# arnaucube/fhe-study

Measured on AMD Instinct MI355X. Metric: NTT/s (N=2^16, 64-bit q) per node; achieved HBM GB/s vs roofline, higher is better.
Workload: dtype u64

## Files before the change

### fhe-study_amd/csrc/bfv32.hip

```cpp
#include "bfv32.hpp"
#include "ntt32_big.hpp"

#include <type_traits>

namespace fhe {

__device__ __forceinline__ u32 mont32(u32 x, u32 y, u32 p, u32 pinv_neg) {
    const u64 t = (u64)x * y;
    const u32 m = (u32)t * pinv_neg;
    return (u32)((t + (u64)m * p) >> 32);
}
__device__ __forceinline__ u64 crt2(u32 rA, u32 rB, u32 pA, u32 pB, Tw32 crt) {
    const u32 rAb = csub_u32(rA, pB);
    const u32 diff = rB - rAb + pB;
    const u32 h = csub_u32(mul_shoup32(diff, crt, pB), pB);
    return (u64)rA + (u64)pA * h;
}

#ifndef FHE_B32_INV_T
#define FHE_B32_INV_T 2
#endif
#ifndef FHE_B32_INV_R
#define FHE_B32_INV_R 1
#endif
#ifndef FHE_B32_FWD_PRELOAD
#define FHE_B32_FWD_PRELOAD 1
#endif
#ifndef FHE_B32_FWD_WAVES
#define FHE_B32_FWD_WAVES 4
#endif
#ifndef FHE_B32_RELIN_WAVES
#define FHE_B32_RELIN_WAVES 4
#endif
#ifndef FHE_B32_FWD2_WAVES
#define FHE_B32_FWD2_WAVES 6
#endif
#ifndef FHE_B32_FWD2_PRELOAD
#define FHE_B32_FWD2_PRELOAD 0
#endif
#ifndef FHE_B32_FWD3_WAVES
#define FHE_B32_FWD3_WAVES 4
#endif
#ifndef FHE_B32_FWD3_RELOAD
#define FHE_B32_FWD3_RELOAD 0
#endif
constexpr int fwd_waves(int npr) { return npr == 2 ? FHE_B32_FWD2_WAVES : npr == 3 ? FHE_B32_FWD3_WAVES : FHE_B32_FWD_WAVES; }
constexpr bool fwd_reload(int npr) { return npr == 3 && FHE_B32_FWD3_RELOAD != 0; }
constexpr bool fwd_preload(int npr) { return npr == 2 ? FHE_B32_FWD2_PRELOAD != 0 : FHE_B32_FWD_PRELOAD != 0; }
#ifndef FHE_B32_PARK_LDS
#define FHE_B32_PARK_LDS 1
#endif
constexpr int kRelinWps = 4;
#ifndef FHE_B32_INV_LOOSE
#define FHE_B32_INV_LOOSE 1
#endif
template <int MODE> constexpr int last_in_of() { return (FHE_B32_INV_LOOSE && MODE != 0) ? 8 : 2; }
template <int MODE, int LB>
__device__ __forceinline__ void inv_block(u32 (&v)[1][16], u32 *lds, const Tw32 *ltw, const Tw32 *gtw, u32 tf, u32 p, u32 p2, u32 bq, u32 blk) {
    if constexpr (FHE_B32_INV_LOOSE && MODE != 0) inv_big_loose<LB, MODE == 2, last_in_of<MODE>()>(v, lds, ltw, gtw, tf, p, bq, 1u, blk);
    else if constexpr (MODE == 0) inv_big<LB>(v, lds, ltw, gtw, tf, p, p2, 1u, blk);
    else if constexpr (MODE == 1) inv_big_direct<LB, false>(v, lds, ltw, gtw, tf, p, p2, 1u, blk);
    else inv_big_direct<LB, true>(v, lds, ltw, gtw, tf, p, p2, 1u, blk);
}
template <int LB>
struct Blk {
    using C = Big32<LB>;
    static constexpr u32 M = C::M, TH = C::TH;
    static constexpr size_t LDS(int tables) { return C::TILE_BYTES + (size_t)tables * C::TW_BYTES; }
    static constexpr int park_lds(int tables, int words, int wps) {
        const long wgs = (4L * wps * 64) / (long)TH;
        const long budget = 160L * 1024 / (wgs < 1 ? 1 : wgs) - 1024;
        const long k = (budget - (long)LDS(tables)) / (8L * (long)TH);
        return k < 0 ? 0 : (k > words ? words : (int)k);
    }
    static constexpr size_t LDS_PARKED(int tables, int words, int wps) { return LDS(tables) + (size_t)park_lds(tables, words, wps) * 8 * TH; }
    static __device__ __forceinline__ Tw32 *table(unsigned char *smem, int i) { return reinterpret_cast<Tw32 *>(smem + C::TILE_BYTES + i * C::TW_BYTES); }
};

template <int LB, int NPR, bool WORD32, bool BELOWP = false>
__global__ __launch_bounds__((Big32<LB>::TH), fwd_waves(NPR)) void bfv32_forward_kernel(Bfv32Args a) {
    static_assert(!BELOWP || WORD32, "words below a 27-bit prime are below 2^32");
    using C = Big32<LB>;
    using K = Blk<LB>;
    extern __shared__ __attribute__((aligned(16))) unsigned char smem_raw[];
    u32 *lds = reinterpret_cast<u32 *>(smem_raw);
    const u32 tf = threadIdx.x;
    const u64 g8 = blockIdx.x / 16;
    const u32 r16 = blockIdx.x % 16;
    const u64 row = g8 * 8 + (r16 & 7u);
    const u32 blk = r16 >> 3;
    if (row >= a.rows) return;
#pragma unroll
    for (int i = 0; i < NPR; i++) stage_tw32_block<C::TH>(K::table(smem_raw, i), a.t.tw_fwd[NPR == 1 ? blockIdx.y : i], C::LTW_N, tf, 1u, blk);
    const u64 *__restrict__ src = a.src + row * K::M;
    typename std::conditional<WORD32, u32, u64>::type x[16];
#pragma unroll
    for (int k = 0; k < 16; k++) x[k] = (typename std::conditional<WORD32, u32, u64>::type)src[(u32)k * C::TH + tf];
    __syncthreads();
#pragma unroll
    for (int i = 0; i < NPR; i++) {
        const u32 pr = NPR == 1 ? blockIdx.y : (u32)i;
        const u32 p = a.t.p[pr], p2 = 2u * p;
        if constexpr (fwd_reload(NPR)) {
            if (i > 0) {
                u64 sa = reinterpret_cast<u64>(src);
// ... 28 lines not shown
    }
}
template <int KIN>
__device__ __forceinline__ void last_stage(u32 &lo, u32 &hi, Tw32 ni, Tw32 w1ni, u32 p) {
    static_assert(2 * KIN <= 16, "the sum of two values below KIN p stays in a word (p < 2^32 / 25)");
    const u32 s = lo + hi, d = lo - hi + (u32)KIN * p;
    lo = csub_u32(mul_shoup32(s, ni, p), p);
    hi = csub_u32(mul_shoup32(d, w1ni, p), p);
}

__device__ __forceinline__ u64 zq_scale_round_int(u64 N, u64 q, u64 mu) {
    u64 a = __umul64hi(N, mu);
    u64 f = N - a * q;
    if (f >= q) { f -= q; a += 1; }
    if (f >= q) { f -= q; a += 1; }
    a += (2 * f >= q);
    u64 r = a - __umul64hi(a, mu) * q;
    r = r >= q ? r - q : r;
    return r >= q ? r - q : r;
}

#ifndef FHE_B32_INT_TAIL
#define FHE_B32_INT_TAIL 1
#endif
__device__ __forceinline__ u64 zq_from_f64_small(double ef, double qf, double qinv, u32 q) {
    const double e = round(ef);
#if FHE_B32_INT_TAIL
    const double k = floor(e * qinv);
    int r = (int)fma(-k, qf, e);
    r += (r >> 31) & (int)q;
    return (u64)min((u32)r, (u32)r - q);
#else
    const double k = rint(e * qinv);
    double r = fma(-k, qf, e);
    r = r < 0.0 ? r + qf : r;
    r = r < 0.0 ? r + qf : r;
    r = r >= qf ? r - qf : r;
    return (u64)(u32)r;
#endif
}
__device__ __forceinline__ double exact_quotient(double N, double den, double rden) {
    const double q0 = N * rden;
    const double r = fma(-q0, den, N);
    return fma(r, rden, q0);
}
template <bool SMALL>
__device__ __forceinline__ u64 scale_round(const Bfv32Args &a, long long v) {
    const double N = a.numf * (double)v;
    const double x = a.rdenf != 0.0 ? exact_quotient(N, a.denf, a.rdenf) : N / a.denf;
    if constexpr (SMALL) return zq_from_f64_small(x, (double)a.q, a.qinvf, (u32)a.q);
    else return zq_from_f64_mu(a.q, a.qmu, round(x));
}

template <int LB, bool INT, bool SMALL>
__global__ __launch_bounds__((Big32<LB>::TH), 4) void bfv32_tensor_inverse_kernel(Bfv32Args a) {
    using C = Big32<LB>;
    using K = Blk<LB>;
    extern __shared__ __attribute__((aligned(16))) unsigned char smem_raw[];
    u32 *lds = reinterpret_cast<u32 *>(smem_raw);
    const u32 tf = threadIdx.x;
    const u64 g8 = blockIdx.x / 24;
    const u32 r24 = blockIdx.x % 24;
    const u64 b = g8 * 8 + (r24 & 7u);
    const u32 which = r24 >> 3;
    if (b >= a.batch) return;
#pragma unroll
    for (int i = 0; i < 4; i++) stage_tw32_block<C::TH>(K::table(smem_raw, i), a.t.tw_inv[i >> 1], C::LTW_N, tf, 1u, (u32)(i & 1));
    __syncthreads();
    auto prime = [&](auto prc) __attribute__((always_inline)) {
        constexpr int pr = decltype(prc)::value;
        const u32 p = a.t.p[pr], p2 = 2u * p, pn = a.pinv_neg[pr];
        const u32 *__restrict__ fw = a.fw + (((u64)pr * a.rows) << (LB + 1));
        auto block = [&](u32 blk, u32 (&v)[1][16]) __attribute__((always_inline)) {
            const u32 off = blk * K::M + tf * 4u;
            auto rowp = [&](u32 w) { return fw + (((u64)w * a.batch + b) << (LB + 1)) + off; };
            const u32 *__restrict__ ra = rowp(which == 2 ? 1 : 0), *__restrict__ rb = rowp(which == 0 ? 2 : 3);
            const u32 *__restrict__ rc = rowp(1), *__restrict__ rd = rowp(2);
#pragma unroll
            for (int j = 0; j < 4; j++) {
                const uint4 xa = *reinterpret_cast<const uint4 *>(ra + j * (K::M / 4)), xb = *reinterpret_cast<const uint4 *>(rb + j * (K::M / 4));
                u32 t[4] = {mont32(xa.x, xb.x, p, pn), mont32(xa.y, xb.y, p, pn), mont32(xa.z, xb.z, p, pn), mont32(xa.w, xb.w, p, pn)};
                if (which == 1) {
                    const uint4 xc = *reinterpret_cast<const uint4 *>(rc + j * (K::M / 4)), xd = *reinterpret_cast<const uint4 *>(rd + j * (K::M / 4));
                    t[0] = csub_u32(t[0] + mont32(xc.x, xd.x, p, pn), p2); t[1] = csub_u32(t[1] + mont32(xc.y, xd.y, p, pn), p2);
                    t[2] = csub_u32(t[2] + mont32(xc.z, xd.z, p, pn), p2); t[3] = csub_u32(t[3] + mont32(xc.w, xd.w, p, pn), p2);
                }
                v[0][4 * j] = t[0]; v[0][4 * j + 1] = t[1]; v[0][4 * j + 2] = t[2]; v[0][4 * j + 3] = t[3];
            }
#ifndef FHE_B32_ABLATE_INV
            inv_block<FHE_B32_INV_T, LB>(v, lds, K::table(smem_raw, 2 * pr + (int)blk), a.t.tw_inv[pr], tf, p, p2, a.t.bq[pr], blk);
#endif
        };
        u32 v0[1][16], v1[1][16];
        block(0u, v0);
        block(1u, v1);
        const Tw32 ni = a.ninv_mont[pr], w1ni = a.w1ninv_mont[pr];
        u64 parked = 0;
        u32 tfe = tf;
        asm volatile("" : "+v"(tfe));
        u64 *po = a.out + ((u64)which * a.batch + b) * K::M + tfe;
        u64 psa = reinterpret_cast<u64>(po);
        asm volatile("" : "+v"(psa));
        const gu64 *ps = reinterpret_cast<const gu64 *>(psa);
        if constexpr (pr == 1) parked = ps[0];
#pragma unroll
        for (int k = 0; k < 16; k++) {
            u32 rl = v0[0][k], rh = v1[0][k];
            last_stage<last_in_of<FHE_B32_INV_T>()>(rl, rh, ni, w1ni, p);
            if constexpr (pr == 0) {
                po[(u32)k * C::TH] = ((u64)rh << 32) | rl;
            } else {
                const u32 loA = (u32)parked, hiA = (u32)(parked >> 32);
                if (k + 1 < 16) parked = ps[(u32)(k + 1) * C::TH];
                const long long lo = (long long)crt2(loA, rl, a.t.p[0], a.t.p[1], a.t.crt);
                const long long hi = (long long)crt2(hiA, rh, a.t.p[0], a.t.p[1], a.t.crt);
#ifndef FHE_B32_ABLATE_EPI
                u64 zl, zh;
                if constexpr (INT) {
                    zl = zq_scale_round_int(a.int_num * (u64)lo, a.q, a.qmu);
                    zh = zq_scale_round_int(a.int_num * (u64)hi, a.q, a.qmu);
                } else {
                    zl = scale_round<SMALL>(a, lo);
                    zh = scale_round<SMALL>(a, hi);
                }
#else
                const u64 zl = (u64)lo, zh = (u64)hi;
#endif
                po[(u32)k * C::TH] = zl >= zh ? zl - zh : (a.q + zl) - zh;
                __builtin_amdgcn_sched_barrier(0);
            }
        }
    };
    prime(std::integral_constant<int, 0>{});
    prime(std::integral_constant<int, 1>{});
}

template <int LB, bool SMALL>
__global__ __launch_bounds__((Big32<LB>::TH), FHE_B32_RELIN_WAVES) void bfv32_relin_inverse_kernel(Bfv32Args a) {
    using C = Big32<LB>;
    using K = Blk<LB>;
    extern __shared__ __attribute__((aligned(16))) unsigned char smem_raw[];
    u32 *lds = reinterpret_cast<u32 *>(smem_raw);
    const u32 tf = threadIdx.x;
    const u64 g8 = blockIdx.x / 16;
    const u32 r16 = blockIdx.x % 16;
    const u64 b = g8 * 8 + (r16 & 7u);
    const u32 o = r16 >> 3;
    if (b >= a.batch) return;
#pragma unroll
    for (int i = 0; i < 6; i++) stage_tw32_block<C::TH>(K::table(smem_raw, i), a.t.tw_inv[i >> 1], C::LTW_N, tf, 1u, (u32)(i & 1));
    __syncthreads();
    const u64 off = ((u64)o * a.batch + b) * K::M + tf;
    u64 *park0 = a.park + off, *park1 = park0 + 2 * a.batch * K::M;
    auto prime = [&](auto prc) __attribute__((always_inline)) {
        constexpr int pr = decltype(prc)::value;
        const u32 p = a.t.p[pr], p2 = 2u * p, pn = a.pinv_neg[pr];
        auto block = [&](u32 blk, u32 (&v)[1][16]) __attribute__((always_inline)) {
            const u32 bo = blk * K::M + tf * 4u;
            const u32 *__restrict__ rx = a.x + (((u64)pr * a.batch + b) << (LB + 1)) + bo;
            const u32 *__restrict__ rk = a.key + (((u64)pr * 2 + o) << (LB + 1)) + bo;
#pragma unroll
            for (int j = 0; j < 4; j++) {
                const uint4 xa = *reinterpret_cast<const uint4 *>(rx + j * (K::M / 4)), xb = *reinterpret_cast<const uint4 *>(rk + j * (K::M / 4));
                v[0][4 * j] = mont32(xa.x, xb.x, p, pn); v[0][4 * j + 1] = mont32(xa.y, xb.y, p, pn);
                v[0][4 * j + 2] = mont32(xa.z, xb.z, p, pn); v[0][4 * j + 3] = mont32(xa.w, xb.w, p, pn);
            }
#ifndef FHE_B32_ABLATE_INV
            inv_block<FHE_B32_INV_R, LB>(v, lds, K::table(smem_raw, 2 * pr + (int)blk), a.t.tw_inv[pr], tf, p, p2, a.t.bq[pr], blk);
#endif
        };
        u32 v0[1][16], v1[1][16];
        block(0u, v0);
        block(1u, v1);
        const Tw32 ni = a.ninv_mont[pr], w1ni = a.w1ninv_mont[pr];
        u64 pk0 = 0, pk1 = 0;
        u64 psa0 = reinterpret_cast<u64>(park0), psa1 = reinterpret_cast<u64>(park1);
        asm volatile("" : "+v"(psa0), "+v"(psa1));
        const gu64 *ps0 = reinterpret_cast<const gu64 *>(psa0), *ps1 = reinterpret_cast<const gu64 *>(psa1);
        constexpr int KL = FHE_B32_PARK_LDS ? K::park_lds(6, 16, kRelinWps) : 0;
        u64 *lpark = reinterpret_cast<u64 *>(smem_raw + K::LDS(6)) + tf;
        auto park0_load = [&](int k) __attribute__((always_inline)) { return k < KL ? lpark[(u32)k * C::TH] : ps0[(u32)k * C::TH]; };
        if constexpr (pr >= 1) pk0 = park0_load(0);
        if constexpr (pr == 2) pk1 = ps1[0];
#pragma unroll
        for (int k = 0; k < 16; k++) {
            u32 r2[2] = {v0[0][k], v1[0][k]};
            last_stage<last_in_of<FHE_B32_INV_R>()>(r2[0], r2[1], ni, w1ni, p);
            if constexpr (pr == 0) {
                if (k < KL) lpark[(u32)k * C::TH] = ((u64)r2[1] << 32) | r2[0];
                else park0[(u32)k * C::TH] = ((u64)r2[1] << 32) | r2[0];
            } else if constexpr (pr == 1) {
                const u32 g0[2] = {(u32)pk0, (u32)(pk0 >> 32)};
                if (k + 1 < 16) pk0 = park0_load(k + 1);
                u32 g1[2];
#pragma unroll
                for (int h = 0; h < 2; h++) {
                    const u32 d = r2[h] - csub_u32(g0[h], p) + p;
                    g1[h] = csub_u32(mul_shoup32(d, a.t.crt, p), p);
                }
                park1[(u32)k * C::TH] = ((u64)g1[1] << 32) | g1[0];
            } else {
                const u32 g0[2] = {(u32)pk0, (u32)(pk0 >> 32)}, g1[2] = {(u32)pk1, (u32)(pk1 >> 32)};
                if (k + 1 < 16) { pk0 = park0_load(k + 1); pk1 = ps1[(u32)(k + 1) * C::TH]; }
                long long R2[2];
#pragma unroll
                for (int h = 0; h < 2; h++) {
                    const u32 a0 = csub_u32(csub_u32(g0[h], p), p);
                    const u32 d = r2[h] - a0 + p;
                    const u32 e = csub_u32(mul_shoup32(d, a.t.crt_ac, p), p);
                    const u32 b1 = csub_u32(g1[h], p);
                    const u32 v2 = csub_u32(mul_shoup32(e - b1 + p, a.t.crt_bc, p), p);
                    R2[h] = (long long)((u64)g0[h] + (u64)a.t.p[0] * g1[h] + a.t.P * v2);
                }
                const long long lo = R2[0], hi = R2[1];
#ifndef FHE_B32_ABLATE_EPI
                const u64 zl = scale_round<SMALL>(a, lo);
                const u64 zh = scale_round<SMALL>(a, hi);
#else
                const u64 zl = (u64)lo, zh = (u64)hi;
#endif
                u64 v = zl >= zh ? zl - zh : (a.q + zl) - zh;
                const u64 at = off + (u32)k * C::TH;
                v += a.addend[at];
                if (v >= a.q) v -= a.q;
                a.out[at] = v;
                __builtin_amdgcn_sched_barrier(0);
            }
        }
    };
    prime(std::integral_constant<int, 0>{});
    prime(std::integral_constant<int, 1>{});
    prime(std::integral_constant<int, 2>{});
}

static unsigned bits_of64(uint64_t x) { unsigned b = 0; while (x) { b++; x >>= 1; } return b; }

bool bfv32_shape_supported(uint64_t q, uint64_t n, uint64_t pq) {
    if (n < 1024 || n > 8192 || (n & (n - 1)) || q < 2) return false;
    const unsigned ln = bits_of64(n - 1), bq = bits_of64(q - 1);
    if (2 * bq + ln + 1 > 54) return false;
    if (pq && (pq < q || bq + bits_of64(pq - 1) + ln > 82)) return false;
    return true;
}

template <typename K>
static hipError_t launch_big(K kernel, const char *name, int lp, size_t lds, unsigned th, u64 grid, const Bfv32Args &a, hipStream_t st,
                             unsigned gridy = 1) {
    if (grid == 0) return hipSuccess;
    if (grid > 0x7fffffffull) return hipErrorInvalidValue;
    if (hipError_t e = allow_big_lds((const void *)kernel, lds)) return e;
    KernelTimer kt(name, lp, st);
    hipLaunchKernelGGL(kernel, dim3((unsigned)grid, gridy), dim3(th), lds, st, a);
    return hipGetLastError();
}
#define FHE_BIG_SWITCH(KERNEL, NAME, GRID, GRIDY, TABLES, PARKW, WPS)                                                               \
    switch (a.log_n2) {                                                                                                      \
        case 11: return launch_big(KERNEL<10>, NAME, 11, Blk<10>::LDS_PARKED(TABLES, PARKW, WPS), Big32<10>::TH, GRID, a, st, GRIDY); \
        case 12: return launch_big(KERNEL<11>, NAME, 12, Blk<11>::LDS_PARKED(TABLES, PARKW, WPS), Big32<11>::TH, GRID, a, st, GRIDY); \
        case 13: return launch_big(KERNEL<12>, NAME, 13, Blk<12>::LDS_PARKED(TABLES, PARKW, WPS), Big32<12>::TH, GRID, a, st, GRIDY); \
        case 14: return launch_big(KERNEL<13>, NAME, 14, Blk<13>::LDS_PARKED(TABLES, PARKW, WPS), Big32<13>::TH, GRID, a, st, GRIDY); \
    }                                                                                                                        \
    return hipErrorNotSupported;

template <int LB> static constexpr auto bfv32_forward2 = bfv32_forward_kernel<LB, 2, true>;
template <int LB> static constexpr auto bfv32_forward3 = bfv32_forward_kernel<LB, 3, true>;
template <int LB> static constexpr auto bfv32_forward2b = bfv32_forward_kernel<LB, 2, true, true>;
template <int LB> static constexpr auto bfv32_forward3b = bfv32_forward_kernel<LB, 3, true, true>;
template <int LB> static constexpr auto bfv32_forward1w = bfv32_forward_kernel<LB, 1, false>;
hipError_t launch_bfv32_forward(const Bfv32Args &a, hipStream_t st) {
    const u64 grid = 16 * ((a.rows + 7) / 8);
    if (a.primes == 2 && a.word32 && a.below_p) { FHE_BIG_SWITCH(bfv32_forward2b, "bfv32_forward", grid, 1, 2, 0, 4) }
    if (a.primes == 3 && a.word32 && a.below_p) { FHE_BIG_SWITCH(bfv32_forward3b, "bfv32_forward3", grid, 1, 3, 0, 4) }
    if (a.primes == 2 && a.word32) { FHE_BIG_SWITCH(bfv32_forward2, "bfv32_forward", grid, 1, 2, 0, 4) }
    if (a.primes == 3 && a.word32) { FHE_BIG_SWITCH(bfv32_forward3, "bfv32_forward3", grid, 1, 3, 0, 4) }
    if (a.primes == 3) { FHE_BIG_SWITCH(bfv32_forward1w, "bfv32_forward_key", grid, 3, 1, 0, 4) }
    return hipErrorNotSupported;
}
template <int LB> static constexpr auto bfv32_tensor_inverse_f64 = bfv32_tensor_inverse_kernel<LB, false, false>;
template <int LB> static constexpr auto bfv32_tensor_inverse_f64s = bfv32_tensor_inverse_kernel<LB, false, true>;
template <int LB> static constexpr auto bfv32_tensor_inverse_int = bfv32_tensor_inverse_kernel<LB, true, false>;
hipError_t launch_bfv32_tensor_inverse(const Bfv32Args &a, hipStream_t st) {
    if (a.int_num) { FHE_BIG_SWITCH(bfv32_tensor_inverse_int, "bfv32_tensor_inverse", 24 * ((a.batch + 7) / 8), 1, 4, 0, 4) }
    if (a.small_f64) { FHE_BIG_SWITCH(bfv32_tensor_inverse_f64s, "bfv32_tensor_inverse", 24 * ((a.batch + 7) / 8), 1, 4, 0, 4) }
    FHE_BIG_SWITCH(bfv32_tensor_inverse_f64, "bfv32_tensor_inverse", 24 * ((a.batch + 7) / 8), 1, 4, 0, 4)
}
template <int LB> static constexpr auto bfv32_relin_inverse_gen = bfv32_relin_inverse_kernel<LB, false>;
template <int LB> static constexpr auto bfv32_relin_inverse_small = bfv32_relin_inverse_kernel<LB, true>;
hipError_t launch_bfv32_relin_inverse(const Bfv32Args &a, hipStream_t st) {
    if (a.small_f64) { FHE_BIG_SWITCH(bfv32_relin_inverse_small, "bfv32_relin_inverse", 16 * ((a.batch + 7) / 8), 1, 6, (FHE_B32_PARK_LDS ? 16 : 0), kRelinWps) }
    FHE_BIG_SWITCH(bfv32_relin_inverse_gen, "bfv32_relin_inverse", 16 * ((a.batch + 7) / 8), 1, 6, (FHE_B32_PARK_LDS ? 16 : 0), kRelinWps)
}
#undef FHE_BIG_SWITCH

bool bfv32_ablated() {
#if defined(FHE_B32_ABLATE_INV) || defined(FHE_B32_ABLATE_EPI)
    return true;
#else
    return false;
#endif
}

}
```

### fhe-study_amd/csrc/bfv32.hpp

```cpp
#pragma once
#include "digit32.hpp"

namespace fhe {

struct Bfv32Args {
    Ext32Args t;
    uint32_t pinv_neg[3];
    Tw32 ninv_mont[3];
    Tw32 w1ninv_mont[3];
    uint32_t log_n2;
    const u64 *src;
    uint32_t *fw;
    u64 rows;
    uint32_t primes;
    uint32_t word32;
    uint32_t below_p;
    const uint32_t *x, *key;
    const u64 *addend;
    u64 *out;
    u64 *park;
    u64 batch, q;
    u64 qmu;
    double numf, denf;
    double rdenf;
    u64 int_num;
    uint32_t small_f64;
    double qinvf;
};

bool bfv32_shape_supported(uint64_t q, uint64_t n, uint64_t pq);
hipError_t launch_bfv32_forward(const Bfv32Args &a, hipStream_t st);
hipError_t launch_bfv32_tensor_inverse(const Bfv32Args &a, hipStream_t st);
hipError_t launch_bfv32_relin_inverse(const Bfv32Args &a, hipStream_t st);

}
```

### fhe-study_amd/csrc/zring.hip

```cpp
#include <cstdio>
#include <cstdlib>
#include <cstring>
#include <map>
#include <vector>

#include "capi_internal.hpp"
#include "digit_mac.hpp"
#include "digit32.hpp"
#include "bfv32.hpp"
#include "ntt_rounds.hpp"
#include "zq_device.hpp"
#include "mac_kernel.hpp"

using fhe::Mod;
using fhe::Tw;
using fhe::u32;
using fhe::u64;
typedef unsigned __int128 u128;

static const u64 kCrtPrimes[3] = {
    2305843009211596801ull,
    2305843009196916737ull,
    2305843009146585089ull,
};
// ... 433 lines not shown
    ZProduct p{};
    p.a = d_a; p.b = d_b; p.a_rows = p.b_rows = p.out_rows = batch; p.n_src = n; p.n = 2 * n;
    p.bits = a_bits + b_bits + ceil_log2(n);
    return z_product(p, d_out, (hipStream_t)hip_stream);
}

extern "C" int fhe_mul_div_round_dev(uint64_t q, uint64_t n, const void *d_v, uint64_t num, uint64_t den,
                                     void *d_out, size_t batch, void *hip_stream) {
    if (n < 1) return fhe_fail(FHE_E_BAD_N, "fhe_mul_div_round_dev: n = 0");
    if (q == 0 || den == 0 || (q >> 63)) return fhe_fail(FHE_E_BAD_Q, "fhe_mul_div_round_dev: q must be in [1, 2^63), den > 0");
    if (batch == 0) return FHE_OK;
    if (!d_v || !d_out) return fhe_fail(FHE_E_NULL, "fhe_mul_div_round_dev: NULL buffer");
    int dev;
    int rc = fhe_current_device(&dev);
    if (rc != FHE_OK) return rc;
    return launch("zr_mul_div_round", 0, (hipStream_t)hip_stream, fhe::zr_mul_div_round_kernel, fhe_ew_grid(batch * n), 256, d_v, d_out, batch, (u32)n, q,
                  num, den);
}

static bool bfv32_on(uint64_t q, uint64_t n, uint64_t pq) { return fhe_ext32_enabled() && fhe::bfv32_shape_supported(q, n, pq); }
static int bfv32_args(uint64_t n, fhe::Bfv32Args *a) {
    int rc = fhe_ext32_tables(2 * n, &a->t);
    if (rc != FHE_OK) return rc;
    a->log_n2 = ceil_log2(2 * n);
    for (int i = 0; i < 3; i++) {
        const uint32_t p = a->t.p[i];
        a->pinv_neg[i] = fhe::host::neg_inv32(p);
        const u64 w = mulmod(a->t.ninv[i].w, 1ull << 32, p);
        a->ninv_mont[i] = tw32(w, p);
        const fhe_ntt_plan *plan = nullptr;
        if ((rc = fhe_ntt_plan_get(p, 2 * n, &plan)) != FHE_OK) return rc;
        a->w1ninv_mont[i] = tw32(mulmod(plan->roots_inv[1], w, p), p);
    }
    return FHE_OK;
}
static bool bfv32_small_f64_on() {
    static const bool on = fhe_env_switch("FHE_BFV_SMALL_F64", true);
    return on;
}
static double bfv32_rden(uint64_t den) {
    static const bool on = fhe_env_switch("FHE_BFV_FAST_DIV", true);
    return (on && (den & 1ull) && den < (1ull << 48)) ? 1.0 / (double)den : 0.0;
}
static uint32_t bfv32_below_p(uint64_t q, const fhe::Bfv32Args &a, int primes) {
    static const bool on = fhe_env_switch("FHE_BFV_BELOW_P", true);
    for (int i = 0; i < primes; i++) if (q > a.t.p[i]) return 0u;
    return on ? 1u : 0u;
}
static int bfv32_tensor(uint64_t q, uint64_t n, uint64_t t, const void *d_ab, void *d_c, size_t batch, hipStream_t st) {
    fhe::Bfv32Args a{};
    int rc = bfv32_args(n, &a);
    if (rc != FHE_OK) return rc;
    void *wsv = nullptr;
    if ((rc = fhe_workspace_get(1, (u64)2 * 4 * batch * 2 * n * 4, st, &wsv)) != FHE_OK) return rc;
    a.src = (const u64 *)d_ab; a.fw = (uint32_t *)wsv; a.rows = 4 * (u64)batch; a.primes = 2; a.word32 = 1;
    a.below_p = bfv32_below_p(q, a, 2);
    if (a.below_p && (rc = fhe_check_canonical_words(q, d_ab, 4 * batch * n, st, "fhe_bfv_tensor_dev")) != FHE_OK) return rc;
    hipError_t e = fhe::launch_bfv32_forward(a, st);
    if (e != hipSuccess) return fhe_hip_fail(e, "bfv32_forward_kernel");
    a.batch = batch; a.out = (u64 *)d_c; a.q = q; a.qmu = ~0ull / q; a.numf = (double)t; a.denf = (double)q;
    a.rdenf = ((unsigned __int128)2 * n * (q - 1) * (q - 1) * t / q < ((unsigned __int128)1 << 52)) ? bfv32_rden(q) : 0.0;
    {
        static const bool on = fhe_env_switch("FHE_BFV_INT_ROUND", false);
        const unsigned __int128 vmax = (unsigned __int128)2 * n * (q - 1) * (q - 1);
        a.int_num = (on && t != 0 && vmax * t < ((unsigned __int128)1 << 52)) ? t : 0;
        a.small_f64 = (bfv32_small_f64_on() && q < (1ull << 30) && vmax * t / q < ((unsigned __int128)1 << 50)) ? 1u : 0u;
        a.qinvf = 1.0 / (double)q;
    }
    e = fhe::launch_bfv32_tensor_inverse(a, st);
    return e == hipSuccess ? FHE_OK : fhe_hip_fail(e, "bfv32_tensor_inverse_kernel");
}
static int bfv32_rlk_prepare(uint64_t n, const u64 *d_rlk, void *prep, hipStream_t st) {
    fhe::Bfv32Args a{};
    int rc = bfv32_args(n, &a);
    if (rc != FHE_OK) return rc;
    a.src = d_rlk; a.fw = (uint32_t *)prep; a.rows = 2; a.primes = 3;
    hipError_t e = fhe::launch_bfv32_forward(a, st);
    return e == hipSuccess ? FHE_OK : fhe_hip_fail(e, "bfv32_forward_kernel");
}
static int bfv32_relinearize(uint64_t q, uint64_t n, uint64_t pq, const void *d_prep, const void *d_c, void *d_out, size_t batch,
                             hipStream_t st) {
    fhe::Bfv32Args a{};
    int rc = bfv32_args(n, &a);
    if (rc != FHE_OK) return rc;
    void *wsv = nullptr;
    const u64 x_bytes = (u64)3 * batch * 2 * n * 4, park_bytes = (u64)2 * 2 * batch * n * 8;
    if ((rc = fhe_workspace_get(1, x_bytes + park_bytes, st, &wsv)) != FHE_OK) return rc;
    a.park = (u64 *)((unsigned char *)wsv + x_bytes);
    a.src = (const u64 *)d_c + 2 * (u64)batch * n; a.fw = (uint32_t *)wsv; a.rows = batch; a.primes = 3; a.word32 = 1;
    a.below_p = bfv32_below_p(q, a, 3);
    if (a.below_p && (rc = fhe_check_canonical_words(q, a.src, batch * n, st, "fhe_bfv_relinearize_dev (c2)")) != FHE_OK) return rc;
    hipError_t e = fhe::launch_bfv32_forward(a, st);
    if (e != hipSuccess) return fhe_hip_fail(e, "bfv32_forward_kernel");
    a.x = (const uint32_t *)wsv; a.key = (const uint32_t *)d_prep;
    a.addend = (const u64 *)d_c; a.out = (u64 *)d_out; a.batch = batch; a.q = q; a.qmu = ~0ull / q; a.numf = 1.0; a.denf = (double)(pq / q);
    a.rdenf = (pq % q == 0 && pq / q >= (1ull << 12)) ? bfv32_rden(pq / q) : 0.0;
    a.small_f64 = (bfv32_small_f64_on() && q < (1ull << 30) && pq / q >= (1ull << 14)) ? 1u : 0u;
    a.qinvf = 1.0 / (double)q;
    e = fhe::launch_bfv32_relin_inverse(a, st);
    return e == hipSuccess ? FHE_OK : fhe_hip_fail(e, "bfv32_relin_inverse_kernel");
}

extern "C" int fhe_bfv_tensor_dev(uint64_t q, uint64_t n, uint64_t t, const void *d_ab, void *d_c, size_t batch,
                                  void *hip_stream) {
    int rc = check_ring(n, "fhe_bfv_tensor_dev");
    if (rc != FHE_OK) return rc;
    if (q < 2 || (q >> 63)) return fhe_fail(FHE_E_BAD_Q, "fhe_bfv_tensor_dev: q must be in [2, 2^63)");
    if (batch == 0) return FHE_OK;
    if (!d_ab || !d_c) return fhe_fail(FHE_E_NULL, "fhe_bfv_tensor_dev: NULL buffer");
    REQUIRE_ALIGNED(d_ab); REQUIRE_ALIGNED(d_c);
    if (bfv32_on(q, n, 0)) return bfv32_tensor(q, n, t, d_ab, d_c, batch, (hipStream_t)hip_stream);
    const u64 n2 = 2 * n;
    ZCtx z;
    rc = zctx_init(&z, n2, primes_for_bits(2 * bits_of(q - 1) + ceil_log2(n) + 1, false));
    if (rc != FHE_OK) return rc;
    hipStream_t st = (hipStream_t)hip_stream;
    const u64 words = batch * n2;
    void *wsv = nullptr;
    rc = fhe_workspace_get(1, (4 + 3 * (size_t)z.K) * words * 8, st, &wsv);
    if (rc != FHE_OK) return rc;
    u64 *AB = (u64 *)wsv, *R = AB + 4 * words;
    for (int k = 0; k < z.K; k++) {
        if ((rc = z_forward_src(z, k, (const u64 *)d_ab, AB, 4 * batch, n, st)) != FHE_OK) return rc;
        u64 *Rk = R + 3 * (u64)k * words;
        if ((rc = launch("zr_tensor", 0, st, fhe::zr_tensor_kernel, fhe_ew_grid(words), 256, AB, Rk, words, z.cc.m[k])) != FHE_OK) return rc;
        if (z.K == 1) {
            hipError_t e = z_inverse_mdr(z, Rk, (u64 *)d_c, 3 * batch, q, t, q, st);
            if (e == hipSuccess) return FHE_OK;
            if (e != hipErrorNotSupported) return fhe_hip_fail(e, "zr_inv_strided_mdr_kernel");
            (void)hipGetLastError();
        }
        if ((rc = z_inverse(z, k, Rk, Rk, 3 * batch, st)) != FHE_OK) return rc;
    }
    return z_crt_mdr(z, R, R + 3 * words, R + 6 * words, nullptr, d_c, 3 * batch, n, q, t, q, st);
}

static unsigned relin_split_bits(uint64_t q, uint64_t n, uint64_t pq) {
    const unsigned h = (bits_of(pq - 1) + 1) / 2;
    return (h >= 1 && bits_of(q - 1) + h + ceil_log2(n) <= 60) ? h : 0;
}
static int bfv_relin_ctx(ZCtx *z, unsigned *h, uint64_t q, uint64_t n, uint64_t pq, const char *who) {
// ... 422 lines not shown
```

Baseline: 2.812 million.

## Split BFV inverse NTT into per-plane block kernels plus separate CRT epilogue

Adds a split path, on by default for relinearization (FHE_B32_SPLIT=2), where each workgroup inverse-transforms a single prime/half plane for one output. Those residues go to a 32-bit workspace with nontemporal stores, and a separate elementwise epilogue kernel then does the CRT/Garner reconstruction, scale-rounding and addend. This exposes more independent workgroups and higher occupancy (8 waves) in place of the serial per-prime loop with parked intermediates. The cost is an extra HBM round trip for the residue planes and an extra kernel launch per tile.

```diff
diff --git a/fhe-study_amd/csrc/bfv32.hip b/fhe-study_amd/csrc/bfv32.hip
--- a/fhe-study_amd/csrc/bfv32.hip
+++ b/fhe-study_amd/csrc/bfv32.hip
@@ -1,6 +1,7 @@
 #include "bfv32.hpp"
 #include "ntt32_big.hpp"
 
+#include <cstdlib>
 #include <type_traits>
 
 namespace fhe {
@@ -50,7 +51,22 @@
 #ifndef FHE_B32_PARK_LDS
 #define FHE_B32_PARK_LDS 1
 #endif
-constexpr int kRelinWps = 4;
+constexpr int kRelinWps = FHE_B32_RELIN_WAVES;
+#ifndef FHE_B32_SPLIT
+#define FHE_B32_SPLIT 2
+#endif
+#ifndef FHE_B32_SPLIT_TILE
+#define FHE_B32_SPLIT_TILE 0
+#endif
+#ifndef FHE_B32_SPLIT_WAVES
+#define FHE_B32_SPLIT_WAVES 8
+#endif
+#ifndef FHE_B32_SPLIT_NT
+#define FHE_B32_SPLIT_NT 1
+#endif
+#ifndef FHE_B32_SPLIT_INV
+#define FHE_B32_SPLIT_INV 2
+#endif
 #ifndef FHE_B32_INV_LOOSE
 #define FHE_B32_INV_LOOSE 1
 #endif
@@ -185,6 +201,43 @@
     else return zq_from_f64_mu(a.q, a.qmu, round(x));
 }
 
+template <int LB>
+__device__ __forceinline__ void tensor_products(u32 (&v)[1][16], const u32 *__restrict__ fw, u64 batch, u64 b, u32 which, u32 off, u32 p, u32 p2, u32 pn) {
+    constexpr u32 Q = Big32<LB>::M / 4;
+    auto rowp = [&](u32 w) { return fw + (((u64)w * batch + b) << (LB + 1)) + off; };
+    const u32 *__restrict__ ra = rowp(which == 2 ? 1 : 0), *__restrict__ rb = rowp(which == 0 ? 2 : 3);
+    const u32 *__restrict__ rc = rowp(1), *__restrict__ rd = rowp(2);
+#pragma unroll
+    for (int j = 0; j < 4; j++) {
+        const uint4 xa = *reinterpret_cast<const uint4 *>(ra + j * Q), xb = *reinterpret_cast<const uint4 *>(rb + j * Q);
+        u32 t[4] = {mont32(xa.x, xb.x, p, pn), mont32(xa.y, xb.y, p, pn), mont32(xa.z, xb.z, p, pn), mont32(xa.w, xb.w, p, pn)};
+        if (which == 1) {
+            const uint4 xc = *reinterpret_cast<const uint4 *>(rc + j * Q), xd = *reinterpret_cast<const uint4 *>(rd + j * Q);
+            t[0] = csub_u32(t[0] + mont32(xc.x, xd.x, p, pn), p2); t[1] = csub_u32(t[1] + mont32(xc.y, xd.y, p, pn), p2);
+            t[2] = csub_u32(t[2] + mont32(xc.z, xd.z, p, pn), p2); t[3] = csub_u32(t[3] + mont32(xc.w, xd.w, p, pn), p2);
+        }
+        v[0][4 * j] = t[0]; v[0][4 * j + 1] = t[1]; v[0][4 * j + 2] = t[2]; v[0][4 * j + 3] = t[3];
+    }
+}
+template <bool INT, bool SMALL>
+__device__ __forceinline__ u64 tensor_coeff(const Bfv32Args &a, u32 loA, u32 hiA, u32 loB, u32 hiB) {
+    const long long lo = (long long)crt2(loA, loB, a.t.p[0], a.t.p[1], a.t.crt);
+    const long long hi = (long long)crt2(hiA, hiB, a.t.p[0], a.t.p[1], a.t.crt);
+#ifndef FHE_B32_ABLATE_EPI
+    u64 zl, zh;
+    if constexpr (INT) {
+        zl = zq_scale_round_int(a.int_num * (u64)lo, a.q, a.qmu);
+        zh = zq_scale_round_int(a.int_num * (u64)hi, a.q, a.qmu);
+    } else {
+        zl = scale_round<SMALL>(a, lo);
+        zh = scale_round<SMALL>(a, hi);
+    }
+#else
+    const u64 zl = (u64)lo, zh = (u64)hi;
+#endif
+    return zl >= zh ? zl - zh : (a.q + zl) - zh;
+}
+
 template <int LB, bool INT, bool SMALL>
 __global__ __launch_bounds__((Big32<LB>::TH), 4) void bfv32_tensor_inverse_kernel(Bfv32Args a) {
     using C = Big32<LB>;
@@ -205,21 +258,7 @@
         const u32 p = a.t.p[pr], p2 = 2u * p, pn = a.pinv_neg[pr];
         const u32 *__restrict__ fw = a.fw + (((u64)pr * a.rows) << (LB + 1));
         auto block = [&](u32 blk, u32 (&v)[1][16]) __attribute__((always_inline)) {
-            const u32 off = blk * K::M + tf * 4u;
-            auto rowp = [&](u32 w) { return fw + (((u64)w * a.batch + b) << (LB + 1)) + off; };
-            const u32 *__restrict__ ra = rowp(which == 2 ? 1 : 0), *__restrict__ rb = rowp(which == 0 ? 2 : 3);
-            const u32 *__restrict__ rc = rowp(1), *__restrict__ rd = rowp(2);
-#pragma unroll
-            for (int j = 0; j < 4; j++) {
-                const uint4 xa = *reinterpret_cast<const uint4 *>(ra + j * (K::M / 4)), xb = *reinterpret_cast<const uint4 *>(rb + j * (K::M / 4));
-                u32 t[4] = {mont32(xa.x, xb.x, p, pn), mont32(xa.y, xb.y, p, pn), mont32(xa.z, xb.z, p, pn), mont32(xa.w, xb.w, p, pn)};
-                if (which == 1) {
-                    const uint4 xc = *reinterpret_cast<const uint4 *>(rc + j * (K::M / 4)), xd = *reinterpret_cast<const uint4 *>(rd + j * (K::M / 4));
-                    t[0] = csub_u32(t[0] + mont32(xc.x, xd.x, p, pn), p2); t[1] = csub_u32(t[1] + mont32(xc.y, xd.y, p, pn), p2);
-                    t[2] = csub_u32(t[2] + mont32(xc.z, xd.z, p, pn), p2); t[3] = csub_u32(t[3] + mont32(xc.w, xd.w, p, pn), p2);
-                }
-                v[0][4 * j] = t[0]; v[0][4 * j + 1] = t[1]; v[0][4 * j + 2] = t[2]; v[0][4 * j + 3] = t[3];
-            }
+            tensor_products<LB>(v, fw, a.batch, b, which, blk * K::M + tf * 4u, p, p2, pn);
 #ifndef FHE_B32_ABLATE_INV
             inv_block<FHE_B32_INV_T, LB>(v, lds, K::table(smem_raw, 2 * pr + (int)blk), a.t.tw_inv[pr], tf, p, p2, a.t.bq[pr], blk);
 #endif
@@ -245,21 +284,7 @@
             } else {
                 const u32 loA = (u32)parked, hiA = (u32)(parked >> 32);
                 if (k + 1 < 16) parked = ps[(u32)(k + 1) * C::TH];
-                const long long lo = (long long)crt2(loA, rl, a.t.p[0], a.t.p[1], a.t.crt);
-                const long long hi = (long long)crt2(hiA, rh, a.t.p[0], a.t.p[1], a.t.crt);
-#ifndef FHE_B32_ABLATE_EPI
-                u64 zl, zh;
-                if constexpr (INT) {
-                    zl = zq_scale_round_int(a.int_num * (u64)lo, a.q, a.qmu);
-                    zh = zq_scale_round_int(a.int_num * (u64)hi, a.q, a.qmu);
-                } else {
-                    zl = scale_round<SMALL>(a, lo);
-                    zh = scale_round<SMALL>(a, hi);
-                }
-#else
-                const u64 zl = (u64)lo, zh = (u64)hi;
-#endif
-                po[(u32)k * C::TH] = zl >= zh ? zl - zh : (a.q + zl) - zh;
+                po[(u32)k * C::TH] = tensor_coeff<INT, SMALL>(a, loA, hiA, rl, rh);
                 __builtin_amdgcn_sched_barrier(0);
             }
         }
@@ -268,6 +293,44 @@
     prime(std::integral_constant<int, 1>{});
 }
 
+template <int LB>
+__device__ __forceinline__ void relin_products(u32 (&v)[1][16], const Bfv32Args &a, u32 pr, u64 b, u32 o, u32 off, u32 p, u32 pn) {
+    constexpr u32 Q = Big32<LB>::M / 4;
+    const u32 *__restrict__ rx = a.x + (((u64)pr * a.batch + b) << (LB + 1)) + off;
+    const u32 *__restrict__ rk = a.key + (((u64)pr * 2 + o) << (LB + 1)) + off;
+#pragma unroll
+    for (int j = 0; j < 4; j++) {
+        const uint4 xa = *reinterpret_cast<const uint4 *>(rx + j * Q), xb = *reinterpret_cast<const uint4 *>(rk + j * Q);
+        v[0][4 * j] = mont32(xa.x, xb.x, p, pn); v[0][4 * j + 1] = mont32(xa.y, xb.y, p, pn);
+        v[0][4 * j + 2] = mont32(xa.z, xb.z, p, pn); v[0][4 * j + 3] = mont32(xa.w, xb.w, p, pn);
+    }
+}
+__device__ __forceinline__ u32 garner_v1(const Ext32Args &t, u32 rB, u32 v0) {
+    const u32 p = t.p[1];
+    const u32 d = rB - csub_u32(v0, p) + p;
+    return csub_u32(mul_shoup32(d, t.crt, p), p);
+}
+__device__ __forceinline__ long long garner_x(const Ext32Args &t, u32 rC, u32 v0, u32 v1) {
+    const u32 p = t.p[2];
+    const u32 a0 = csub_u32(csub_u32(v0, p), p);
+    const u32 d = rC - a0 + p;
+    const u32 e = csub_u32(mul_shoup32(d, t.crt_ac, p), p);
+    const u32 b1 = csub_u32(v1, p);
+    const u32 v2 = csub_u32(mul_shoup32(e - b1 + p, t.crt_bc, p), p);
+    return (long long)((u64)v0 + (u64)t.p[0] * v1 + t.P * v2);
+}
+template <bool SMALL>
+__device__ __forceinline__ u64 relin_coeff(const Bfv32Args &a, long long lo, long long hi, u64 addend) {
+#ifndef FHE_B32_ABLATE_EPI
+    const u64 zl = scale_round<SMALL>(a, lo);
+    const u64 zh = scale_round<SMALL>(a, hi);
+#else
+    const u64 zl = (u64)lo, zh = (u64)hi;
+#endif
+    u64 v = zl >= zh ? zl - zh : (a.q + zl) - zh;
+    v += addend;
+    return v >= a.q ? v - a.q : v;
+}
 template <int LB, bool SMALL>
 __global__ __launch_bounds__((Big32<LB>::TH), FHE_B32_RELIN_WAVES) void bfv32_relin_inverse_kernel(Bfv32Args a) {
     using C = Big32<LB>;
@@ -289,15 +352,7 @@
         constexpr int pr = decltype(prc)::value;
         const u32 p = a.t.p[pr], p2 = 2u * p, pn = a.pinv_neg[pr];
         auto block = [&](u32 blk, u32 (&v)[1][16]) __attribute__((always_inline)) {
-            const u32 bo = blk * K::M + tf * 4u;
-            const u32 *__restrict__ rx = a.x + (((u64)pr * a.batch + b) << (LB + 1)) + bo;
-            const u32 *__restrict__ rk = a.key + (((u64)pr * 2 + o) << (LB + 1)) + bo;
-#pragma unroll
-            for (int j = 0; j < 4; j++) {
-                const uint4 xa = *reinterpret_cast<const uint4 *>(rx + j * (K::M / 4)), xb = *reinterpret_cast<const uint4 *>(rk + j * (K::M / 4));
-                v[0][4 * j] = mont32(xa.x, xb.x, p, pn); v[0][4 * j + 1] = mont32(xa.y, xb.y, p, pn);
-                v[0][4 * j + 2] = mont32(xa.z, xb.z, p, pn); v[0][4 * j + 3] = mont32(xa.w, xb.w, p, pn);
-            }
+            relin_products<LB>(v, a, (u32)pr, b, o, blk * K::M + tf * 4u, p, pn);
 #ifndef FHE_B32_ABLATE_INV
             inv_block<FHE_B32_INV_R, LB>(v, lds, K::table(smem_raw, 2 * pr + (int)blk), a.t.tw_inv[pr], tf, p, p2, a.t.bq[pr], blk);
 #endif
@@ -325,38 +380,13 @@
             } else if constexpr (pr == 1) {
                 const u32 g0[2] = {(u32)pk0, (u32)(pk0 >> 32)};
                 if (k + 1 < 16) pk0 = park0_load(k + 1);
-                u32 g1[2];
-#pragma unroll
-                for (int h = 0; h < 2; h++) {
-                    const u32 d = r2[h] - csub_u32(g0[h], p) + p;
-                    g1[h] = csub_u32(mul_shoup32(d, a.t.crt, p), p);
-                }
+                const u32 g1[2] = {garner_v1(a.t, r2[0], g0[0]), garner_v1(a.t, r2[1], g0[1])};
                 park1[(u32)k * C::TH] = ((u64)g1[1] << 32) | g1[0];
             } else {
                 const u32 g0[2] = {(u32)pk0, (u32)(pk0 >> 32)}, g1[2] = {(u32)pk1, (u32)(pk1 >> 32)};
                 if (k + 1 < 16) { pk0 = park0_load(k + 1); pk1 = ps1[(u32)(k + 1) * C::TH]; }
-                long long R2[2];
-#pragma unroll
-                for (int h = 0; h < 2; h++) {
-                    const u32 a0 = csub_u32(csub_u32(g0[h], p), p);
-                    const u32 d = r2[h] - a0 + p;
-                    const u32 e = csub_u32(mul_shoup32(d, a.t.crt_ac, p), p);
-                    const u32 b1 = csub_u32(g1[h], p);
-                    const u32 v2 = csub_u32(mul_shoup32(e - b1 + p, a.t.crt_bc, p), p);
-                    R2[h] = (long long)((u64)g0[h] + (u64)a.t.p[0] * g1[h] + a.t.P * v2);
-                }
-                const long long lo = R2[0], hi = R2[1];
-#ifndef FHE_B32_ABLATE_EPI
-                const u64 zl = scale_round<SMALL>(a, lo);
-                const u64 zh = scale_round<SMALL>(a, hi);
-#else
-                const u64 zl = (u64)lo, zh = (u64)hi;
-#endif
-                u64 v = zl >= zh ? zl - zh : (a.q + zl) - zh;
                 const u64 at = off + (u32)k * C::TH;
-                v += a.addend[at];
-                if (v >= a.q) v -= a.q;
-                a.out[at] = v;
+                a.out[at] = relin_coeff<SMALL>(a, garner_x(a.t, r2[0], g0[0], g1[0]), garner_x(a.t, r2[1], g0[1], g1[1]), a.addend[at]);
                 __builtin_amdgcn_sched_barrier(0);
             }
         }
@@ -364,6 +394,115 @@
     prime(std::integral_constant<int, 0>{});
     prime(std::integral_constant<int, 1>{});
     prime(std::integral_constant<int, 2>{});
+}
+
+template <u32 OUTS, u32 PLANES>
+struct SplitId {
+    u64 bt;
+    u32 out, pr, blk;
+    __device__ __forceinline__ SplitId(u32 id) {
+        constexpr u32 S = OUTS * PLANES;
+        const u32 r = id % (8 * S), s = r >> 3;
+        bt = (u64)(id / (8 * S)) * 8 + (r & 7u);
+        out = s % OUTS;
+        pr = (s / OUTS) >> 1;
+        blk = (s / OUTS) & 1u;
+    }
+    static u64 grid(u64 pairs) { return 8ull * OUTS * PLANES * ((pairs + 7) / 8); }
+};
+template <int LB, u32 OUTS, u32 PLANES>
+__device__ __forceinline__ void store_plane(const Bfv32Args &a, const SplitId<OUTS, PLANES> &w, const u32 (&v)[1][16], u32 tf) {
+    u32 *__restrict__ dst = a.res + (((w.bt * OUTS + w.out) * PLANES + 2 * w.pr + w.blk) << LB) + tf;
+#pragma unroll
+    for (int k = 0; k < 16; k++) {
+#if FHE_B32_SPLIT_NT
+        __builtin_nontemporal_store(v[0][k], dst + (u32)k * Big32<LB>::TH);
+#else
+        dst[(u32)k * Big32<LB>::TH] = v[0][k];
+#endif
+    }
+}
+template <int LB, bool RELIN>
+__global__ __launch_bounds__((Big32<LB>::TH), FHE_B32_SPLIT_WAVES) void bfv32_block_inverse_kernel(Bfv32Args a) {
+    using C = Big32<LB>;
+    using K = Blk<LB>;
+    using Id = SplitId<RELIN ? 2u : 3u, RELIN ? 6u : 4u>;
+    extern __shared__ __attribute__((aligned(16))) unsigned char smem_raw[];
+    u32 *lds = reinterpret_cast<u32 *>(smem_raw);
+    const u32 tf = threadIdx.x;
+    const Id w(blockIdx.x);
+    if (w.bt >= a.tile_pairs) return;
+    const u64 b = a.tile0 + w.bt;
+    stage_tw32_block<C::TH>(K::table(smem_raw, 0), a.t.tw_inv[w.pr], C::LTW_N, tf, 1u, w.blk);
+    const u32 p = a.t.p[w.pr], p2 = 2u * p, pn = a.pinv_neg[w.pr];
+    u32 v[1][16];
+    if constexpr (RELIN) relin_products<LB>(v, a, w.pr, b, w.out, w.blk * K::M + tf * 4u, p, pn);
+    else tensor_products<LB>(v, a.fw + (((u64)w.pr * a.rows) << (LB + 1)), a.batch, b, w.out, w.blk * K::M + tf * 4u, p, p2, pn);
+    __syncthreads();
+#ifndef FHE_B32_ABLATE_INV
+    inv_block<FHE_B32_SPLIT_INV, LB>(v, lds, K::table(smem_raw, 0), a.t.tw_inv[w.pr], tf, p, p2, a.t.bq[w.pr], w.blk);
+#endif
+    store_plane<LB>(a, w, v, tf);
+}
+template <int LB>
+__device__ __forceinline__ void split_residues(const Bfv32Args &a, const u32 *__restrict__ pl, int pr, u32 (&lo)[4], u32 (&hi)[4]) {
+#if FHE_B32_SPLIT_NT
+    typedef u32 v4u __attribute__((ext_vector_type(4)));
+    const v4u x0 = __builtin_nontemporal_load(reinterpret_cast<const v4u *>(pl + ((u64)(2 * pr) << LB))), x1 = __builtin_nontemporal_load(reinterpret_cast<const v4u *>(pl + ((u64)(2 * pr + 1) << LB)));
+#else
+    const uint4 x0 = *reinterpret_cast<const uint4 *>(pl + ((u64)(2 * pr) << LB)), x1 = *reinterpret_cast<const uint4 *>(pl + ((u64)(2 * pr + 1) << LB));
+#endif
+    lo[0] = x0.x; lo[1] = x0.y; lo[2] = x0.z; lo[3] = x0.w;
+    hi[0] = x1.x; hi[1] = x1.y; hi[2] = x1.z; hi[3] = x1.w;
+#pragma unroll
+    for (int e = 0; e < 4; e++) last_stage<last_in_of<FHE_B32_SPLIT_INV>()>(lo[e], hi[e], a.ninv_mont[pr], a.w1ninv_mont[pr], a.t.p[pr]);
+}
+template <int LB, bool INT, bool SMALL>
+__global__ __launch_bounds__(256) void bfv32_tensor_epilogue_kernel(Bfv32Args a) {
+    const u64 i = (u64)blockIdx.x * 256 + threadIdx.x;
+    const u64 row = i >> (LB - 2);
+    if (row >= 3 * a.tile_pairs) return;
+    const u32 j = ((u32)i & ((1u << (LB - 2)) - 1u)) * 4u;
+    const u64 bt = row / 3;
+    const u32 which = (u32)(row - 3 * bt);
+    const u32 *__restrict__ pl = a.res + ((row * 4) << LB) + j;
+    u32 loA[4], hiA[4], loB[4], hiB[4];
+    split_residues<LB>(a, pl, 0, loA, hiA);
+    split_residues<LB>(a, pl, 1, loB, hiB);
+    u64 z[4];
+#pragma unroll
+    for (int e = 0; e < 4; e++) z[e] = tensor_coeff<INT, SMALL>(a, loA[e], hiA[e], loB[e], hiB[e]);
+    ulonglong2 *po = reinterpret_cast<ulonglong2 *>(a.out + (((u64)which * a.batch + a.tile0 + bt) << LB) + j);
+    po[0] = make_ulonglong2(z[0], z[1]);
+    po[1] = make_ulonglong2(z[2], z[3]);
+}
+template <int LB, bool SMALL>
+__global__ __launch_bounds__(256) void bfv32_relin_epilogue_kernel(Bfv32Args a) {
+    const u64 i = (u64)blockIdx.x * 256 + threadIdx.x;
+    const u64 row = i >> (LB - 2);
+    if (row >= 2 * a.tile_pairs) return;
+    const u32 j = ((u32)i & ((1u << (LB - 2)) - 1u)) * 4u;
+    const u64 bt = row >> 1;
+    const u32 o = (u32)row & 1u;
+    const u32 *__restrict__ pl = a.res + ((row * 6) << LB) + j;
+    const u64 at = (((u64)o * a.batch + a.tile0 + bt) << LB) + j;
+    const ulonglong2 *pa = reinterpret_cast<const ulonglong2 *>(a.addend + at);
+    const ulonglong2 ad0 = pa[0], ad1 = pa[1];
+    const u64 ad[4] = {ad0.x, ad0.y, ad1.x, ad1.y};
+    u32 lo0[4], hi0[4], lo1[4], hi1[4], lo2[4], hi2[4];
+    split_residues<LB>(a, pl, 0, lo0, hi0);
+    split_residues<LB>(a, pl, 1, lo1, hi1);
+    split_residues<LB>(a, pl, 2, lo2, hi2);
+    u64 z[4];
+#pragma unroll
+    for (int e = 0; e < 4; e++) {
+        const long long lo = garner_x(a.t, lo2[e], lo0[e], garner_v1(a.t, lo1[e], lo0[e]));
+        const long long hi = garner_x(a.t, hi2[e], hi0[e], garner_v1(a.t, hi1[e], hi0[e]));
+        z[e] = relin_coeff<SMALL>(a, lo, hi, ad[e]);
+    }
+    ulonglong2 *po = reinterpret_cast<ulonglong2 *>(a.out + at);
+    po[0] = make_ulonglong2(z[0], z[1]);
+    po[1] = make_ulonglong2(z[2], z[3]);
 }
 
 static unsigned bits_of64(uint64_t x) { unsigned b = 0; while (x) { b++; x >>= 1; } return b; }
@@ -409,10 +548,69 @@
     if (a.primes == 3) { FHE_BIG_SWITCH(bfv32_forward1w, "bfv32_forward_key", grid, 3, 1, 0, 4) }
     return hipErrorNotSupported;
 }
+static unsigned split_mask() {
+    static const unsigned m = [] {
+        const char *e = getenv("FHE_B32_SPLIT");
+        return (e && e[0] >= '0' && e[0] <= '3' && !e[1]) ? (unsigned)(e[0] - '0') : (unsigned)(FHE_B32_SPLIT);
+    }();
+    return m;
+}
+static u64 split_tile(u64 batch) {
+    static const u64 tile = [] {
+        const char *e = getenv("FHE_B32_SPLIT_TILE");
+        return e ? (u64)strtoull(e, nullptr, 10) : (u64)(FHE_B32_SPLIT_TILE);
+    }();
+    return (tile == 0 || tile > batch) ? batch : tile;
+}
+u64 bfv32_split_res_bytes(bool relin, uint64_t n, u64 batch) {
+    if (!(split_mask() & (relin ? 2u : 1u))) return 0;
+    return split_tile(batch) * 12 * n * 4;
+}
+template <class B, class E>
+static hipError_t launch_split(B block, E epilogue, Bfv32Args a, u32 outs) {
+    if (!a.res) return hipErrorInvalidValue;
+    const u64 batch = a.batch, tile = split_tile(batch);
+    for (a.tile0 = 0; a.tile0 < batch; a.tile0 += tile) {
+        a.tile_pairs = batch - a.tile0 < tile ? batch - a.tile0 : tile;
+        if (hipError_t e = block(a, 8ull * 12 * ((a.tile_pairs + 7) / 8))) return e;
+        if (hipError_t e = epilogue(a, (outs * a.tile_pairs << (a.log_n2 - 3)) / 256)) return e;
+    }
+    return hipSuccess;
+}
+template <int LB> static constexpr auto bfv32_tensor_block_inverse = bfv32_block_inverse_kernel<LB, false>;
+template <int LB> static constexpr auto bfv32_relin_block_inverse = bfv32_block_inverse_kernel<LB, true>;
+template <int LB> static constexpr auto bfv32_tensor_epilogue_f64 = bfv32_tensor_epilogue_kernel<LB, false, false>;
+template <int LB> static constexpr auto bfv32_tensor_epilogue_f64s = bfv32_tensor_epilogue_kernel<LB, false, true>;
+template <int LB> static constexpr auto bfv32_tensor_epilogue_int = bfv32_tensor_epilogue_kernel<LB, true, false>;
+template <int LB> static constexpr auto bfv32_relin_epilogue_gen = bfv32_relin_epilogue_kernel<LB, false>;
+template <int LB> static constexpr auto bfv32_relin_epilogue_small = bfv32_relin_epilogue_kernel<LB, true>;
+static hipError_t launch_tensor_block(const Bfv32Args &a, u64 grid, hipStream_t st) { FHE_BIG_SWITCH(bfv32_tensor_block_inverse, "bfv32_tensor_inverse", grid, 1, 1, 0, 4) }
+static hipError_t launch_relin_block(const Bfv32Args &a, u64 grid, hipStream_t st) { FHE_BIG_SWITCH(bfv32_relin_block_inverse, "bfv32_relin_inverse", grid, 1, 1, 0, 4) }
+#define FHE_EPI_SWITCH(KERNEL, NAME)                                                              \
+    switch (a.log_n2) {                                                                           \
+        case 11: return launch_big(KERNEL<10>, NAME, 11, 0, 256, grid, a, st);                    \
+        case 12: return launch_big(KERNEL<11>, NAME, 12, 0, 256, grid, a, st);                    \
+        case 13: return launch_big(KERNEL<12>, NAME, 13, 0, 256, grid, a, st);                    \
+        case 14: return launch_big(KERNEL<13>, NAME, 14, 0, 256, grid, a, st);                    \
+    }                                                                                             \
+    return hipErrorNotSupported;
+static hipError_t launch_tensor_epilogue(const Bfv32Args &a, u64 grid, hipStream_t st) {
+    if (a.int_num) { FHE_EPI_SWITCH(bfv32_tensor_epilogue_int, "bfv32_tensor_epilogue") }
+    if (a.small_f64) { FHE_EPI_SWITCH(bfv32_tensor_epilogue_f64s, "bfv32_tensor_epilogue") }
+    FHE_EPI_SWITCH(bfv32_tensor_epilogue_f64, "bfv32_tensor_epilogue")
+}
+static hipError_t launch_relin_epilogue(const Bfv32Args &a, u64 grid, hipStream_t st) {
+    if (a.small_f64) { FHE_EPI_SWITCH(bfv32_relin_epilogue_small, "bfv32_relin_epilogue") }
+    FHE_EPI_SWITCH(bfv32_relin_epilogue_gen, "bfv32_relin_epilogue")
+}
+#undef FHE_EPI_SWITCH
 template <int LB> static constexpr auto bfv32_tensor_inverse_f64 = bfv32_tensor_inverse_kernel<LB, false, false>;
 template <int LB> static constexpr auto bfv32_tensor_inverse_f64s = bfv32_tensor_inverse_kernel<LB, false, true>;
 template <int LB> static constexpr auto bfv32_tensor_inverse_int = bfv32_tensor_inverse_kernel<LB, true, false>;
 hipError_t launch_bfv32_tensor_inverse(const Bfv32Args &a, hipStream_t st) {
+    if (split_mask() & 1u)
+        return launch_split([st](const Bfv32Args &t, u64 g) { return launch_tensor_block(t, g, st); },
+                            [st](const Bfv32Args &t, u64 g) { return launch_tensor_epilogue(t, g, st); }, a, 3);
     if (a.int_num) { FHE_BIG_SWITCH(bfv32_tensor_inverse_int, "bfv32_tensor_inverse", 24 * ((a.batch + 7) / 8), 1, 4, 0, 4) }
     if (a.small_f64) { FHE_BIG_SWITCH(bfv32_tensor_inverse_f64s, "bfv32_tensor_inverse", 24 * ((a.batch + 7) / 8), 1, 4, 0, 4) }
     FHE_BIG_SWITCH(bfv32_tensor_inverse_f64, "bfv32_tensor_inverse", 24 * ((a.batch + 7) / 8), 1, 4, 0, 4)
@@ -420,6 +618,9 @@
 template <int LB> static constexpr auto bfv32_relin_inverse_gen = bfv32_relin_inverse_kernel<LB, false>;
 template <int LB> static constexpr auto bfv32_relin_inverse_small = bfv32_relin_inverse_kernel<LB, true>;
 hipError_t launch_bfv32_relin_inverse(const Bfv32Args &a, hipStream_t st) {
+    if (split_mask() & 2u)
+        return launch_split([st](const Bfv32Args &t, u64 g) { return launch_relin_block(t, g, st); },
+                            [st](const Bfv32Args &t, u64 g) { return launch_relin_epilogue(t, g, st); }, a, 2);
     if (a.small_f64) { FHE_BIG_SWITCH(bfv32_relin_inverse_small, "bfv32_relin_inverse", 16 * ((a.batch + 7) / 8), 1, 6, (FHE_B32_PARK_LDS ? 16 : 0), kRelinWps) }
     FHE_BIG_SWITCH(bfv32_relin_inverse_gen, "bfv32_relin_inverse", 16 * ((a.batch + 7) / 8), 1, 6, (FHE_B32_PARK_LDS ? 16 : 0), kRelinWps)
 }
diff --git a/fhe-study_amd/csrc/bfv32.hpp b/fhe-study_amd/csrc/bfv32.hpp
--- a/fhe-study_amd/csrc/bfv32.hpp
+++ b/fhe-study_amd/csrc/bfv32.hpp
@@ -19,6 +19,8 @@
     const u64 *addend;
     u64 *out;
     u64 *park;
+    uint32_t *res;
+    u64 tile0, tile_pairs;
     u64 batch, q;
     u64 qmu;
     double numf, denf;
@@ -29,6 +31,7 @@
 };
 
 bool bfv32_shape_supported(uint64_t q, uint64_t n, uint64_t pq);
+u64 bfv32_split_res_bytes(bool relin, uint64_t n, u64 batch);
 hipError_t launch_bfv32_forward(const Bfv32Args &a, hipStream_t st);
 hipError_t launch_bfv32_tensor_inverse(const Bfv32Args &a, hipStream_t st);
 hipError_t launch_bfv32_relin_inverse(const Bfv32Args &a, hipStream_t st);
diff --git a/fhe-study_amd/csrc/zring.hip b/fhe-study_amd/csrc/zring.hip
--- a/fhe-study_amd/csrc/zring.hip
+++ b/fhe-study_amd/csrc/zring.hip
@@ -509,7 +509,9 @@
     int rc = bfv32_args(n, &a);
     if (rc != FHE_OK) return rc;
     void *wsv = nullptr;
-    if ((rc = fhe_workspace_get(1, (u64)2 * 4 * batch * 2 * n * 4, st, &wsv)) != FHE_OK) return rc;
+    const u64 fw_bytes = (u64)2 * 4 * batch * 2 * n * 4;
+    if ((rc = fhe_workspace_get(1, fw_bytes + fhe::bfv32_split_res_bytes(false, n, batch), st, &wsv)) != FHE_OK) return rc;
+    a.res = (uint32_t *)((unsigned char *)wsv + fw_bytes);
     a.src = (const u64 *)d_ab; a.fw = (uint32_t *)wsv; a.rows = 4 * (u64)batch; a.primes = 2; a.word32 = 1;
     a.below_p = bfv32_below_p(q, a, 2);
     if (a.below_p && (rc = fhe_check_canonical_words(q, d_ab, 4 * batch * n, st, "fhe_bfv_tensor_dev")) != FHE_OK) return rc;
@@ -541,9 +543,11 @@
     int rc = bfv32_args(n, &a);
     if (rc != FHE_OK) return rc;
     void *wsv = nullptr;
-    const u64 x_bytes = (u64)3 * batch * 2 * n * 4, park_bytes = (u64)2 * 2 * batch * n * 8;
+    const u64 x_bytes = (u64)3 * batch * 2 * n * 4, res_bytes = fhe::bfv32_split_res_bytes(true, n, batch);
+    const u64 park_bytes = res_bytes ? res_bytes : (u64)2 * 2 * batch * n * 8;
     if ((rc = fhe_workspace_get(1, x_bytes + park_bytes, st, &wsv)) != FHE_OK) return rc;
     a.park = (u64 *)((unsigned char *)wsv + x_bytes);
+    a.res = (uint32_t *)a.park;
     a.src = (const u64 *)d_c + 2 * (u64)batch * n; a.fw = (uint32_t *)wsv; a.rows = batch; a.primes = 3; a.word32 = 1;
     a.below_p = bfv32_below_p(q, a, 3);
     if (a.below_p && (rc = fhe_check_canonical_words(q, a.src, batch * n, st, "fhe_bfv_relinearize_dev (c2)")) != FHE_OK) return rc;
```

Result: no change. 2.810 million (median of 2 runs) (-0.0%).
